# arnauqb/GradABM-JUNE

Measured on NVIDIA B200. Metric: agent_timesteps_per_sec_fwd_bwd, higher is better.
Workload: dtype f32

## Files before the change

### gradabm-june_b200/csrc/gj_kernels.cu

```cuda
#include <cuda_runtime.h>
#include <math.h>
#include <stdint.h>
#include <stdio.h>
#include <stdlib.h>
#include <string.h>

#include "gj_device.cuh"
#include "gj_tiled.cuh"
#include "gj_lean.cuh"
#include "gj_pipe.cuh"

namespace gj {

static thread_local char g_err[512] = "";

static int fail(const char* what, cudaError_t e) {
  snprintf(g_err, sizeof(g_err), "%s: %s", what, cudaGetErrorString(e));
  return -2;
}
static int bad(const char* what) {
  snprintf(g_err, sizeof(g_err), "invalid argument: %s", what);
  return -1;
}
#define GJ_CHECK_LAUNCH(name)                         \
// ... 559 lines not shown
         aligned16(w->orig_id) &&
         aligned16(lp.r_slot) && aligned16(lp.r_pc);
}
static bool pipe_aligned_bwd(const gj_world_desc* w, const LeanPlan& lp, const gj_bwd_io* io) {
  const void* ptrs[] = {io->s, io->inf, io->tinf, io->cur, io->nxt, io->ttn, io->tape_y0, io->tape_v, io->g_s_o,
                        io->g_inf_o, io->g_tinf_o, io->g_cur_o, io->g_nxt_o, io->g_ttn_o, io->prof4, io->g_inf,
                        io->g_tinf, io->T_in, io->w, io->wq, w->ent1, w->cls, lp.r_slot, lp.r_pc};
  for (const void* q : ptrs)
    if (!aligned16(q)) return false;
  return true;
}
template <typename K>
static int pipe_grid(const gj_world_desc* w, K kernel, int threads, size_t smem, OccCache* cache,
                     const Batch& bt = kNoBatch) {
  int& c = cache->v[current_device()];
  if (c == 0) {
    int per_sm = 0;
    cudaFuncSetAttribute(kernel, cudaFuncAttributeMaxDynamicSharedMemorySize, (int)smem);
    if (cudaOccupancyMaxActiveBlocksPerMultiprocessor(&per_sm, kernel, threads, smem) != cudaSuccess || per_sm < 1)
      per_sm = 1;
    c = per_sm;
  }
  const int64_t g = (int64_t)sm_count() * c;
  if (bt.nb > 1) return batch_grid(w, g, bt);
  return (int)(w->n_tiles < g ? w->n_tiles : g);
}

static int check_world(const gj_world_desc* w) {
  if (!w) return bad("world is NULL");
  if (w->n_agents < 0 || w->n_types < 0 || w->n_types > GJ_MAX_TYPES) return bad("world sizes");
  if (w->n_edges >= ((int64_t)1 << 32) || w->n_agents >= ((int64_t)1 << 32)) return bad("world too large for 32-bit CSR");
  for (int t = 0; t < w->n_types; ++t)
    if (w->type_group_off[t + 1] - w->type_group_off[t] >= ((int64_t)1 << 28)) return bad("too many groups in one type");
  return 0;
}

template <bool kBwd>
static int launch_group_pass(const gj_world_desc* w, const gj_step_params* p, const Channels& ch, const float* beta,
                             const float* lprob, const float* in0, const float* in1, float* out_a, float* out_b,
                             const Scratch& sc, cudaStream_t st) {
  if (w->n_small > 0) {
    ProfScope ps(kBwd ? K_GROUP_SMALL_B : K_GROUP_SMALL_F, st);
    k_group_small<kBwd><<<blocks_for(w->n_small, kBlock), kBlock, 0, st>>>(*w, *p, ch, beta, lprob, in0, in1, out_a,
                                                                         out_b);
    GJ_CHECK_LAUNCH("k_group_small");
  }
  if (w->n_chunks > 0) {
    ProfScope ps(kBwd ? K_GROUP_CHUNK_B : K_GROUP_CHUNK_F, st);
    k_group_chunk<kBwd><<<blocks_for(w->n_chunks * 32, kBlock), kBlock, 0, st>>>(*w, *p, ch, beta, lprob, in0, in1,
                                                                              out_a, out_b, sc.part_a, sc.part_b);
    GJ_CHECK_LAUNCH("k_group_chunk");
  }
  if (w->n_big > 0) {
    ProfScope ps(kBwd ? K_GROUP_FIX_B : K_GROUP_FIX_F, st);
    k_group_fix<kBwd><<<blocks_for(w->n_big, kBlock), kBlock, 0, st>>>(*w, *p, ch, beta, sc.part_a, sc.part_b, out_a,
                                                                     out_b);
    GJ_CHECK_LAUNCH("k_group_fix");
  }
  return 0;
}

static int launch_cell_groups(const gj_world_desc* w, const gj_step_params* p, const Plan& pl, const float* beta,
                              float* out_scaled, float* out_plain, const Scratch& sc, cudaStream_t st,
                              const Batch& bt = kNoBatch) {
  if (pl.n_t2 == 0) return 0;
  int64_t maxG = 1;
// ... 47 lines not shown
      lp->c_row[j] = p->nets[k].prob_row;
      lp->c_care[j] = kind == GJ_KIND_CARE_VISIT;
      lp->c_cell_off[j] = w->cell_off[t];
      lp->c_tile_cell[j] = w->tile_cell[t];
      bool seen = false;
      for (int i = 0; i < lp->n_tc; ++i) seen = seen || lp->tc[i] == w->tile_cell[t];
      if (!seen) {
        lp->ctp[lp->n_tc] = w->cell_tile_ptr[t];
        lp->tc[lp->n_tc++] = w->tile_cell[t];
      }
    } else if (kind == GJ_KIND_HOUSEHOLD) {
      if (p->n_quar > 0) return false;
    } else if (kind != GJ_KIND_PLAIN) {
      return false;
    }
  }
  lp->n_cell = pl.n_t2;
  lp->has_generic = pl.n_generic > 0;
  lp->gen_base = total;
  return true;
}

static int launch_lean_group_pass(const gj_world_desc* w, const gj_step_params* p, const Plan& pl, const float* beta,
                                  const float* in, float* out_scaled, float* out_plain, const Scratch& sc, bool bwd,
                                  cudaStream_t st, const Batch& bt);
static int launch_lean_forward_sums(const gj_world_desc* w, const gj_step_params* p, const Plan& pl, const float* beta,
                                    const float* in, float* out_scaled, float* out_plain, const Scratch& sc,
                                    cudaStream_t st, const Batch& bt) {
  if (w->n_giant_chunks > 0) {
    gj_world_desc wg = *w;
    wg.n_small = 0;
    wg.n_chunks = w->n_giant_chunks;
    wg.n_big = w->n_giant_big;
    if (int e = launch_lean_group_pass(&wg, p, pl, beta, in, out_scaled, out_plain, sc, false, st, bt)) return e;
  }
  {
    ProfScope ps(K_GROUP_SMALL_F, st);
    Scatter sct{sc.sct_acc, sc.sct_dirty};
    GenericRanges gr;
    memset(&gr, 0, sizeof(gr));
    for (int t = 0; t < w->n_types; ++t)
      if (w->type_tier[t] == GJ_TIER_GENERIC && w->type_group_off[t + 1] > w->type_group_off[t]) {
        gr.first[gr.n] = w->type_group_off[t];
        gr.start[gr.n + 1] = gr.start[gr.n] + (w->type_group_off[t + 1] - w->type_group_off[t]);
        ++gr.n;
      }
    if (gr.n == 0) return 0;
    launch_pdl(k_lean_scatter_finalize, dim3(blocks_for(gr.start[gr.n], kBlock) * bt.nb), dim3(kBlock), 0, st, *w, *p, pl,
               gr, beta, in, sct, out_scaled, out_plain, bt);
    GJ_CHECK_LAUNCH("k_lean_scatter_finalize");
  }
  return 0;
}

static int launch_lean_group_pass(const gj_world_desc* w, const gj_step_params* p, const Plan& pl, const float* beta,
                                  const float* in, float* out_scaled, float* out_plain, const Scratch& sc, bool bwd,
                                  cudaStream_t st, const Batch& bt) {
  if (w->n_small > 0 || w->n_chunks > 0) {
    ProfScope ps(bwd ? K_GROUP_CHUNK_B : K_GROUP_CHUNK_F, st);
    const int chunk_blocks = w->n_chunks > 0 ? blocks_for(w->n_chunks * 32, kBlock) : 0;
    const int small_blocks = w->n_small > 0 ? blocks_for(w->n_small, kBlock) : 0;
    launch_pdl(k_lean_group_sums, dim3((chunk_blocks + small_blocks) * bt.nb), dim3(kBlock), 0, st, *w, *p, pl, beta, in,
               out_scaled, out_plain, sc.part_a, chunk_blocks, bt);
    GJ_CHECK_LAUNCH("k_lean_group_sums");
  }
  if (w->n_big > 0) {
    ProfScope ps(bwd ? K_GROUP_FIX_B : K_GROUP_FIX_F, st);
    launch_pdl(k_lean_group_fix, dim3(blocks_for(w->n_big * 32, kBlock) * bt.nb), dim3(kBlock), 0, st, *w, *p, pl, beta,
               (const float*)sc.part_a, out_scaled, out_plain, bt);
    GJ_CHECK_LAUNCH("k_lean_group_fix");
  }
  return 0;
}

static int lean_forward(const gj_world_desc* w, const gj_step_params* p, const Plan& pl, const LeanPlan& lp,
                        const gj_fwd_io* io, const Scratch& sc, cudaStream_t st, const NextStep* next,
                        const Batch& bt = kNoBatch) {
  const bool quar = p->n_quar > 0;
  const bool batch = bt.nb > 1;
  if (p->stage != GJ_STAGE_REST) {
    if (!p->t_ready) {
      ProfScope ps(K_TRANSMISSION, st);
      static OccCache occ[4];
      const Scatter sct{sc.sct_acc, sc.sct_dirty};
#define GJ_K1(Q, B, I)                                                                                               \
  launch_pdl(k_lean_transmission<Q, B>, dim3(lean_grid(w, k_lean_transmission<Q, B>, &occ[I], bt)), dim3(kLeanThreads), \
             0, st, *w, *p, lp, *io, sc.tile_part, sct, bt)
#define GJ_K1C(Q, B, I)                                                                                              \
  launch_pdl(k_lean_transmission_c<Q, B>, dim3(lean_grid(w, k_lean_transmission_c<Q, B>, &occ_c[I], bt)),              \
             dim3(kLeanThreads), 0, st, *w, *p, lp, *io, sc.tile_part, sct, bt)
      static OccCache occ_c[4];
      const bool compact = (pipe_flags() & 4) == 0;
      if (compact) {
        if (batch) {
          if (quar) GJ_K1C(true, true, 3);
          else GJ_K1C(false, true, 2);
// ... 811 lines not shown
```

### gradabm-june_b200/csrc/gj_lean.cuh

```cuda
#pragma once
#include "gj_tiled.cuh"

namespace gj {

constexpr int kLeanThreads = 256;
#ifndef GJ_LEAN_MINB_FWD
#define GJ_LEAN_MINB_FWD 3
#endif
#ifndef GJ_LEAN_MINB_BWD
#define GJ_LEAN_MINB_BWD 4
#endif
#ifndef GJ_LEAN_MINB_GATHER
#define GJ_LEAN_MINB_GATHER 3
#endif
constexpr uint32_t kEntNone = 0xFFFFFFFFu;
constexpr uint32_t kEntMulti = 0xFFFFFFFEu;
constexpr uint32_t kEntGiant = 0x80000000u;
constexpr uint32_t kEntId = 0x7FFFFFFFu;

struct Scatter {
  unsigned long long* acc;
  uint8_t* dirty;
};
constexpr float kScatterScale = (float)(1ull << GJ_SCATTER_FRAC);
// ... 434 lines not shown
__device__ __forceinline__ void lean_group_chunk_body(const gj_world_desc& w, const LeanGroupShared& gs, int64_t ci,
                                                      const float* __restrict__ in, float* __restrict__ out_scaled,
                                                      float* __restrict__ out_plain, float* __restrict__ part) {
  const int lane = threadIdx.x & 31;
  if (ci >= w.n_chunks) return;
  const uint32_t g = w.chunk_group[ci];
  const float b = lean_group_beta(gs, g);
  float S = 0.0f;
  if (b == b) {
    const uint32_t j0 = w.chunk_begin[ci], j1 = w.chunk_end[ci];
    constexpr int kDeep = 4;
    for (uint32_t j = j0 + lane; j < j1; j += 32 * kDeep) {
      uint32_t m[kDeep];
      float x[kDeep];
#pragma unroll
      for (int k = 0; k < kDeep; ++k) m[k] = (j + 32 * k < j1) ? w.gm_agent[j + 32 * k] : 0u;
#pragma unroll
      for (int k = 0; k < kDeep; ++k) x[k] = (j + 32 * k < j1) ? in[m[k]] : 0.0f;
#pragma unroll
      for (int k = 0; k < kDeep; ++k) S += x[k];
    }
    S = warp_sum(S);
  }
  if (lane != 0) return;
  const int pi = w.chunk_part[ci];
  if (pi < 0) {
    out_plain[g] = S;
    out_scaled[g] = (b == b) ? (b * w.pc[g]) * S : 0.0f;
  } else {
    part[pi] = S;
  }
}

__global__ void __launch_bounds__(kBlock) k_lean_group_sums(gj_world_desc w, gj_step_params p, Plan pl,
                                                            const float* __restrict__ beta,
                                                            const float* __restrict__ in, float* __restrict__ out_scaled,
                                                            float* __restrict__ out_plain, float* __restrict__ part,
                                                            int chunk_blocks, Batch bt) {
  __shared__ LeanGroupShared gs;
  pdl_launch();
  pdl_wait();
  uint32_t bx = blockIdx.x;
  if (bt.nb > 1) {
    const int s = (int)(bx % (uint32_t)bt.nb);
    bx /= (uint32_t)bt.nb;
    beta += (int64_t)s * bt.sBeta;
    in += (int64_t)s * bt.sN;
    out_scaled += (int64_t)s * bt.sG;
    out_plain += (int64_t)s * bt.sG;
    part = scr_shift(part, bt, s);
  }
  lean_beta_sums(gs, w, p, pl, beta);
  if ((int)bx < chunk_blocks)
    lean_group_chunk_body(w, gs, ((int64_t)bx * blockDim.x + threadIdx.x) >> 5, in, out_scaled, out_plain, part);
  else
    lean_group_small_body(w, gs, (int64_t)(bx - chunk_blocks) * blockDim.x + threadIdx.x, in, out_scaled,
                          out_plain);
}

__global__ void __launch_bounds__(kBlock) k_lean_group_fix(gj_world_desc w, gj_step_params p, Plan pl,
                                                           const float* __restrict__ beta,
                                                           const float* __restrict__ part,
                                                           float* __restrict__ out_scaled,
                                                           float* __restrict__ out_plain, Batch bt) {
  __shared__ LeanGroupShared gs;
  pdl_launch();
  pdl_wait();
  uint32_t bx = blockIdx.x;
  if (bt.nb > 1) {
    const int s = (int)(bx % (uint32_t)bt.nb);
    bx /= (uint32_t)bt.nb;
    beta += (int64_t)s * bt.sBeta;
    out_scaled += (int64_t)s * bt.sG;
    out_plain += (int64_t)s * bt.sG;
    part = scr_shift(part, bt, s);
  }
  lean_beta_sums(gs, w, p, pl, beta);
  const int lane = threadIdx.x & 31;
  const int64_t i = ((int64_t)bx * blockDim.x + threadIdx.x) >> 5;
  if (i >= w.n_big) return;
  const uint32_t g = w.big_groups[i];
  const float b = lean_group_beta(gs, g);
  float S = 0.0f;
  for (uint32_t j = w.big_part_ptr[i] + lane; j < w.big_part_ptr[i + 1]; j += 32) S += part[j];
  S = warp_sum(S);
  if (lane != 0) return;
  out_plain[g] = S;
  out_scaled[g] = (b == b) ? (b * w.pc[g]) * S : 0.0f;
}

// ... 597 lines not shown
```

### gradabm-june_b200/csrc/gj_world.cu

```cuda
#include <cuda_runtime.h>
#include <stdint.h>
#include <stdio.h>
#include <string.h>

#include <string>
#include <vector>

#include <thrust/adjacent_difference.h>
#include <thrust/binary_search.h>
#include <thrust/copy.h>
#include <thrust/count.h>
#include <thrust/device_ptr.h>
#include <thrust/device_vector.h>
#include <thrust/extrema.h>
#include <thrust/fill.h>
#include <thrust/gather.h>
#include <thrust/host_vector.h>
#include <thrust/iterator/counting_iterator.h>
#include <thrust/iterator/zip_iterator.h>
#include <thrust/tuple.h>
#include <thrust/reduce.h>
#include <thrust/scan.h>
#include <thrust/scatter.h>
#include <thrust/sequence.h>
// ... 108 lines not shown
    thrust::copy(b.begin(), b.end(), out.begin() + a.size());
    return out;
  }
  static I64 select(const I64& v, const I64& mask) { return gather(v, nonzero(mask)); }
  static I64 unique_inverse(const I64& keys, int64_t* n_unique) {
    const int64_t n = (int64_t)keys.size();
    I64 k = keys;
    I64 perm = arange(n);
    thrust::sort_by_key(k.begin(), k.end(), perm.begin());
    I64 fresh(n, 0);
    if (n > 0) {
      thrust::transform(k.begin() + 1, k.end(), k.begin(), fresh.begin() + 1,
                        [] __host__ __device__(int64_t a, int64_t b) { return (int64_t)(a != b); });
      thrust::inclusive_scan(fresh.begin(), fresh.end(), fresh.begin());
    }
    I64 rank(n);
    thrust::scatter(fresh.begin(), fresh.end(), perm.begin(), rank.begin());
    *n_unique = n > 0 ? (int64_t)fresh.back() + 1 : 0;
    return rank;
  }
};

struct TypeSrc {
  std::string name;
  int64_t E, G;
};

template <class B>
struct World {
  template <class T>
  using vec = typename B::template vec<T>;
  gj_world_desc desc;
  vec<uint32_t> am_ptr, am_ent, gm_ptr, gm_agent, small_groups, chunk_group, chunk_begin, chunk_end, big_groups,
      big_part_ptr, tile_begin, tile_flags, ent1, orig_id;
  vec<int32_t> chunk_part;
  vec<float> pc;
  vec<uint8_t> cls;
  vec<uint32_t> range_slot[GJ_MAX_TYPES];
  vec<float> range_pc[GJ_MAX_TYPES];
  vec<uint32_t> tile_cell[GJ_MAX_TYPES], cell_tile_ptr[GJ_MAX_TYPES], cell_grp_ptr[GJ_MAX_TYPES], cell_grp[GJ_MAX_TYPES],
      grp_cell_ptr[GJ_MAX_TYPES], grp_cell[GJ_MAX_TYPES];
  vec<int64_t> perm;
  std::string error;
};

template <class B>
struct Builder {
  using O = Ops<B>;
  using I64 = typename O::I64;
  template <class T>
  using vec = typename B::template vec<T>;

  static vec<uint32_t> to_u32(const I64& v, int slack = 0) {
    vec<uint32_t> out(v.size() + slack, 0u);
    thrust::transform(v.begin(), v.end(), out.begin(), [] __host__ __device__(int64_t x) { return (uint32_t)x; });
    return out;
  }
  template <class T>
  static const T* raw(const vec<T>& v) {
    return v.empty() ? nullptr : thrust::raw_pointer_cast(v.data());
  }

  struct Cell {
    int64_t n_cells = 0;
    I64 cell_start, cell_of_agent, cell_grp_ptr, cell_grp, grp_cell_ptr, grp_cell;
  };

// ... 291 lines not shown
  for (int t = 0; t < nt; ++t) {
    if (s->want_tier) want[t] = s->want_tier[t];
    else if (t == range_type) want[t] = GJ_TIER_RANGE;
    else if (t == cell_type) want[t] = GJ_TIER_CELL;
  }
  std::vector<typename Bd::Cell> cells(nt);
  std::vector<int> tier(nt, GJ_TIER_GENERIC);
  I64 g_src, g_key, g_ent;
  for (int t = 0; t < nt; ++t) {
    if (n > 0 && want[t] == GJ_TIER_RANGE) {
      I64 slot;
      typename B::template vec<float> rpc;
      bool from_size = false;
      if (Bd::try_range(n, src[t], dst[t], types[t].G, W->pc, offs[t], &slot, &rpc, &from_size)) {
        tier[t] = GJ_TIER_RANGE;
        d.range_pc_from_size[t] = from_size ? 1 : 0;
        W->range_slot[t] = Bd::to_u32(slot, 32);
        W->range_pc[t] = rpc;
      }
    } else if (n > 0 && want[t] == GJ_TIER_CELL) {
      if (Bd::try_cell(n, src[t], dst[t], types[t].G, &cells[t])) tier[t] = GJ_TIER_CELL;
    }
    if (tier[t] == GJ_TIER_GENERIC) {
      const int64_t off = offs[t], tt = t;
      g_src = O::cat(g_src, src[t]);
      g_key = O::cat(g_key, O::map1(dst[t], [off] __host__ __device__(int64_t g) { return g + off; }));
      g_ent = O::cat(g_ent, O::map1(dst[t], [tt] __host__ __device__(int64_t g) { return g + (tt << 28); }));
    }
  }
  const int64_t E = (int64_t)g_src.size();

  I64 size = O::bincount(g_key, G);
  I64 gm_ptr = O::ptr_from_counts(size);
  {
    I64 perm = O::argsort_stable(g_key);
    W->gm_agent = Bd::to_u32(O::gather(g_src, perm));
  }
  I64 deg = O::bincount(g_src, n);
  I64 am_ptr = O::ptr_from_counts(deg);
  {
    I64 perm = O::argsort_stable(g_src);
    W->am_ent = Bd::to_u32(O::gather(g_ent, perm), 32);
  }
  {
    I64 ent1(n, kNoSlot);
    I64 v = O::map2(g_key, O::gather(size, g_key), [scatter_max] __host__ __device__(int64_t k, int64_t sz) {
      return k + ((int64_t)(sz > scatter_max) << 31);
    });
    O::scatter(ent1, g_src, v);
    thrust::transform(ent1.begin(), ent1.end(), deg.begin(), ent1.begin(),
                      [] __host__ __device__(int64_t e, int64_t dg) { return dg > 1 ? kEntMulti : e; });
    W->ent1 = Bd::to_u32(ent1, 32);
  }
  {
    typename B::template vec<uint8_t> cls(n + 64, (uint8_t)0);
    thrust::transform(sex.begin(), sex.end(), age.begin(), cls.begin(),
                      [] __host__ __device__(int64_t sx, int64_t ag) { return (uint8_t)(sx * 100 + ag); });
    W->cls = cls;
  }

  I64 generic_group(G, 0);
  for (int t = 0; t < nt; ++t)
    if (tier[t] == GJ_TIER_GENERIC) thrust::fill(generic_group.begin() + offs[t], generic_group.begin() + offs[t + 1], (int64_t)1);
  I64 gids = O::arange(G);
  I64 small_mask = O::map2(size, generic_group, [small_group] __host__ __device__(int64_t sz, int64_t g) { return (int64_t)(sz <= small_group && g); });
  I64 big_giant = O::map2(size, generic_group, [small_group, scatter_max] __host__ __device__(int64_t sz, int64_t g) { return (int64_t)(sz > small_group && sz > scatter_max && g); });
  I64 big_rest = O::map2(size, generic_group, [small_group, scatter_max] __host__ __device__(int64_t sz, int64_t g) { return (int64_t)(sz > small_group && sz <= scatter_max && g); });
  I64 small = O::select(gids, small_mask);
  I64 bg_g = O::select(gids, big_giant);
  I64 bg = O::cat(bg_g, O::select(gids, big_rest));
  const int64_t n_giant_big = (int64_t)bg_g.size();
  I64 nchunk = O::map1(O::gather(size, bg), [chunk] __host__ __device__(int64_t sz) { return (sz + chunk - 1) / chunk; });
  int64_t n_giant_chunks = 0;
  if (n_giant_big > 0) n_giant_chunks = thrust::reduce(nchunk.begin(), nchunk.begin() + n_giant_big, (int64_t)0);
  I64 cfirst = O::ptr_from_counts(nchunk);
  I64 cseg = O::segments(cfirst);
  I64 chunk_group = O::gather(bg, cseg);
  const int64_t n_chunks = (int64_t)chunk_group.size();
  I64 within = O::map2(O::arange(n_chunks), O::gather(cfirst, cseg), [] __host__ __device__(int64_t i, int64_t f) { return i - f; });
  I64 chunk_begin = O::map2(O::gather(gm_ptr, chunk_group), within, [chunk] __host__ __device__(int64_t p, int64_t w) { return p + w * chunk; });
  I64 cg1 = O::map1(chunk_group, [] __host__ __device__(int64_t g) { return g + 1; });
  I64 chunk_end = O::map2(chunk_begin, O::gather(gm_ptr, cg1), [chunk] __host__ __device__(int64_t b, int64_t e) { return b + chunk < e ? b + chunk : e; });
  I64 multi_g = O::map1(nchunk, [] __host__ __device__(int64_t c) { return (int64_t)(c > 1); });
  I64 multi = O::gather(multi_g, cseg);
  I64 part_idx(n_chunks, 0);
  thrust::exclusive_scan(multi.begin(), multi.end(), part_idx.begin());
  const int64_t n_parts = O::sum_of(multi);
  {
    typename B::template vec<int32_t> chunk_part(n_chunks);
    thrust::transform(multi.begin(), multi.end(), part_idx.begin(), chunk_part.begin(),
                      [] __host__ __device__(int64_t m, int64_t i) { return m ? (int32_t)i : (int32_t)-1; });
    W->chunk_part = chunk_part;
  }
  I64 big_groups = O::select(bg, multi_g);
  I64 big_part_ptr = O::ptr_from_counts(O::select(nchunk, multi_g));

  I64 cuts(1, 0);
  for (int t = 0; t < nt; ++t)
    if (tier[t] == GJ_TIER_CELL) cuts = O::cat(cuts, cells[t].cell_start);
  I64 tile_begin;
  if (n > 0) {
    thrust::sort(cuts.begin(), cuts.end());
    cuts.resize(thrust::unique(cuts.begin(), cuts.end()) - cuts.begin());
    I64 seg_start = cuts;
    I64 seg_end(seg_start.size());
    thrust::copy(seg_start.begin() + 1, seg_start.end(), seg_end.begin());
    seg_end[seg_end.size() - 1] = n;
    const int64_t T = GJ_TILE_AGENTS;
    I64 ntile = O::map2(seg_end, seg_start, [T] __host__ __device__(int64_t e, int64_t b) { return (e - b + T - 1) / T; });
    I64 tfirst = O::ptr_from_counts(ntile);
    I64 tseg = O::segments(tfirst);
    const int64_t n_tiles = (int64_t)tseg.size();
    I64 tw = O::map2(O::arange(n_tiles), O::gather(tfirst, tseg), [] __host__ __device__(int64_t i, int64_t f) { return i - f; });
    tile_begin = O::map2(O::gather(seg_start, tseg), tw, [T] __host__ __device__(int64_t b, int64_t w) { return b + w * T; });
    tile_begin.push_back(n);
  } else {
    tile_begin = I64(1, 0);
  }
  const int64_t n_tiles = (int64_t)tile_begin.size() - 1;
  I64 tile_flags(n_tiles, 0);
  if (n_tiles > 0) tile_flags[0] = 1;
  int64_t cell_off = 0;
  for (int t = 0; t < nt; ++t) {
    d.type_tier[t] = tier[t];
    d.cell_off[t] = cell_off;
    if (tier[t] == GJ_TIER_RANGE) {
      d.range_slot[t] = Bd::raw(W->range_slot[t]);
      d.range_pc[t] = Bd::raw(W->range_pc[t]);
// ... 5 lines not shown
        thrust::transform(thrust::make_zip_iterator(thrust::make_tuple(tc.begin() + 1, tc.begin(), tile_flags.begin() + 1)),
                          thrust::make_zip_iterator(thrust::make_tuple(tc.end(), tc.end() - 1, tile_flags.end())),
                          tile_flags.begin() + 1, [] __host__ __device__(thrust::tuple<int64_t, int64_t, int64_t> x) {
                            return thrust::get<2>(x) | (int64_t)(thrust::get<0>(x) != thrust::get<1>(x));
                          });
      W->tile_cell[t] = Bd::to_u32(tc);
      I64 ctp = O::searchsorted_left(tb0, c.cell_start);
      ctp.push_back(n_tiles);
      W->cell_tile_ptr[t] = Bd::to_u32(ctp);
      W->cell_grp_ptr[t] = Bd::to_u32(c.cell_grp_ptr);
      W->cell_grp[t] = Bd::to_u32(c.cell_grp);
      W->grp_cell_ptr[t] = Bd::to_u32(c.grp_cell_ptr);
      W->grp_cell[t] = Bd::to_u32(c.grp_cell);
      d.n_cells[t] = c.n_cells;
      d.tile_cell[t] = Bd::raw(W->tile_cell[t]);
      d.cell_tile_ptr[t] = Bd::raw(W->cell_tile_ptr[t]);
      d.cell_grp_ptr[t] = Bd::raw(W->cell_grp_ptr[t]);
      d.cell_grp[t] = Bd::raw(W->cell_grp[t]);
      d.grp_cell_ptr[t] = Bd::raw(W->grp_cell_ptr[t]);
      d.grp_cell[t] = Bd::raw(W->grp_cell[t]);
      cell_off += c.n_cells;
    }
  }
  d.n_cells_total = cell_off;

  W->am_ptr = Bd::to_u32(am_ptr, 32);
  W->gm_ptr = Bd::to_u32(gm_ptr);
  W->small_groups = Bd::to_u32(small);
  W->chunk_group = Bd::to_u32(chunk_group);
  W->chunk_begin = Bd::to_u32(chunk_begin);
  W->chunk_end = Bd::to_u32(chunk_end);
  W->big_groups = Bd::to_u32(big_groups);
  W->big_part_ptr = Bd::to_u32(big_part_ptr);
  W->tile_begin = Bd::to_u32(tile_begin, 4);
  W->tile_flags = Bd::to_u32(tile_flags, 4);
  if (!orig.empty()) W->orig_id = Bd::to_u32(orig, 32);

  d.n_agents = n;
  d.n_groups = G;
  d.n_edges = n_edges_total;
  d.n_types = nt;
  for (int t = 0; t <= nt; ++t) d.type_group_off[t] = offs[t];
  d.am_ptr = Bd::raw(W->am_ptr);
  d.am_ent = Bd::raw(W->am_ent);
  d.gm_ptr = Bd::raw(W->gm_ptr);
  d.gm_agent = Bd::raw(W->gm_agent);
  d.pc = Bd::raw(W->pc);
  d.cls = Bd::raw(W->cls);
  d.small_groups = Bd::raw(W->small_groups);
  d.n_small = (int64_t)small.size();
  d.chunk_group = Bd::raw(W->chunk_group);
  d.chunk_begin = Bd::raw(W->chunk_begin);
  d.chunk_end = Bd::raw(W->chunk_end);
  d.chunk_part = Bd::raw(W->chunk_part);
  d.n_chunks = n_chunks;
  d.big_groups = Bd::raw(W->big_groups);
  d.big_part_ptr = Bd::raw(W->big_part_ptr);
  d.n_big = (int64_t)big_groups.size();
  d.n_parts = n_parts;
  d.n_tiles = n_tiles;
  d.tile_begin = Bd::raw(W->tile_begin);
  d.tile_flags = Bd::raw(W->tile_flags);
  d.ent1 = Bd::raw(W->ent1);
  d.n_giant_chunks = n_giant_chunks;
  d.n_giant_big = n_giant_big;
  d.dbeta_w = nullptr;
  d.orig_id = Bd::raw(W->orig_id);
  (void)E;
  return 0;
}

}

struct gj_world {
  gjw::World<gjw::DeviceBackend>* dev = nullptr;
  gjw::World<gjw::HostBackend>* host = nullptr;
  thrust::host_vector<int64_t> perm_host;
};

static thread_local char g_world_err[512] = "";

extern "C" {

const char* gj_world_last_error(void) { return g_world_err; }

static int build_any(const gj_world_src* src, gj_world** out, bool on_device) {
  if (!src || !out) {
    snprintf(g_world_err, sizeof(g_world_err), "gj_world_build: NULL argument");
    return -1;
  }
  gj_world* w = new gj_world();
  int rc = 0;
// ... 62 lines not shown
```

### gradabm-june_b200/grad_june/_lib.py

```python
import ctypes as C
import os
import subprocess
from pathlib import Path

PKG_DIR = Path(__file__).resolve().parent
CSRC_DIR = PKG_DIR.parent / "csrc"
INCLUDE_DIR = PKG_DIR.parent.parent / "include"
LIB_PATH = Path(os.environ.get("GJ_LIB_PATH") or PKG_DIR / "libgradjune_b200.so")

GJ_MAX_TYPES = 8
GJ_MAX_NETS = 16
GJ_MAX_STAGES = 16
GJ_MAX_QUAR = 4
GJ_MAX_AGE_BINS = 8
GJ_MAX_CHANNELS = 8
GJ_ABI_VERSION = 10

KIND_PLAIN, KIND_HOUSEHOLD, KIND_LEISURE, KIND_CARE_VISIT = 0, 1, 2, 3
PHASE_NETWORKS, PHASE_SAMPLE, PHASE_INFECT, PHASE_SYMPTOMS, PHASE_ALL = 1, 2, 4, 8, 15
MODE_STEP, MODE_SEED = 0, 1
STAGE_ALL, STAGE_SUMS, STAGE_REST = 0, 1, 2

_u32p = C.c_void_p
_f32p = C.c_void_p


class WorldDesc(C.Structure):
    _fields_ = [
        ("n_agents", C.c_int64), ("n_groups", C.c_int64), ("n_edges", C.c_int64),
        ("n_types", C.c_int32), ("_pad0", C.c_int32),
        ("type_group_off", C.c_int64 * (GJ_MAX_TYPES + 1)),
        ("am_ptr", _u32p), ("am_ent", _u32p), ("gm_ptr", _u32p), ("gm_agent", _u32p),
        ("pc", _f32p), ("cls", C.c_void_p),
        ("small_groups", _u32p), ("n_small", C.c_int64),
        ("chunk_group", _u32p), ("chunk_begin", _u32p), ("chunk_end", _u32p), ("chunk_part", C.c_void_p),
        ("n_chunks", C.c_int64),
        ("big_groups", _u32p), ("big_part_ptr", _u32p), ("n_big", C.c_int64), ("n_parts", C.c_int64),
        ("type_tier", C.c_int32 * GJ_MAX_TYPES),
        ("range_slot", C.c_void_p * GJ_MAX_TYPES), ("range_pc", C.c_void_p * GJ_MAX_TYPES),
        ("range_pc_from_size", C.c_int32 * GJ_MAX_TYPES),
        ("n_tiles", C.c_int64), ("tile_begin", _u32p), ("tile_flags", _u32p),
        ("n_cells", C.c_int64 * GJ_MAX_TYPES), ("cell_off", C.c_int64 * GJ_MAX_TYPES), ("n_cells_total", C.c_int64),
        ("tile_cell", C.c_void_p * GJ_MAX_TYPES), ("cell_tile_ptr", C.c_void_p * GJ_MAX_TYPES),
        ("cell_grp_ptr", C.c_void_p * GJ_MAX_TYPES), ("cell_grp", C.c_void_p * GJ_MAX_TYPES),
        ("grp_cell_ptr", C.c_void_p * GJ_MAX_TYPES), ("grp_cell", C.c_void_p * GJ_MAX_TYPES),
        ("ent1", _u32p), ("n_giant_chunks", C.c_int64), ("n_giant_big", C.c_int64), ("dbeta_w", _f32p), ("orig_id", _u32p),
    ]


class WorldSrc(C.Structure):
    _fields_ = [
        ("n_agents", C.c_int64), ("n_types", C.c_int32), ("renumber", C.c_int32),
        ("type_name", C.c_char_p * GJ_MAX_TYPES),
        ("edge_agent", C.c_void_p * GJ_MAX_TYPES), ("edge_group", C.c_void_p * GJ_MAX_TYPES),
        ("n_edges", C.c_int64 * GJ_MAX_TYPES), ("n_groups", C.c_int64 * GJ_MAX_TYPES),
        ("people_i64", C.c_void_p * GJ_MAX_TYPES), ("people_f32", C.c_void_p * GJ_MAX_TYPES),
        ("age", C.c_void_p), ("sex", C.c_void_p), ("original_index", C.c_void_p), ("want_tier", C.c_void_p),
    ]


class Net(C.Structure):
    _fields_ = [("type", C.c_int32), ("kind", C.c_int32), ("prob_row", C.c_int32), ("s_off", C.c_int32)]


class Dist(C.Structure):
    _fields_ = [("kind", C.c_int32), ("loc", C.c_float), ("scale", C.c_float)]


class StepParams(C.Structure):
    _fields_ = [
# ... 199 lines not shown
```

### gradabm-june_b200/grad_june/world.py

```python
import io
import pickle
import sys
from typing import Dict, List, Optional

import numpy as np
import torch

MAX_TYPES = 8


class _Store:
    def __init__(self, key=None):
        object.__setattr__(self, "_mapping", {})
        object.__setattr__(self, "_key", key)

    def __getattr__(self, name):
        if name.startswith("__"):
            raise AttributeError(name)
        mapping = self.__dict__.get("_mapping", {})
        if name in mapping:
            return mapping[name]
        raise AttributeError(f"{type(self).__name__} {self.__dict__.get('_key')!r} has no attribute {name!r}")

    def __setattr__(self, name, value):
# ... 151 lines not shown


def load_world(path_or_file):
    if hasattr(path_or_file, "read"):
        return _WorldUnpickler(path_or_file).load()
    with open(path_or_file, "rb") as f:
        return _WorldUnpickler(f).load()


def world_from_arrays(arrays: Dict[str, np.ndarray], types: List[str], device="cpu") -> HeteroData:
    data = HeteroData()
    n = len(arrays["age"])
    data["agent"].id = torch.arange(n)
    data["agent"].age = torch.as_tensor(np.asarray(arrays["age"]).astype(np.int64))
    data["agent"].sex = torch.as_tensor(np.asarray(arrays["sex"]).astype(np.int64))
    if "ethnicity" in arrays:
        data["agent"].ethnicity = np.asarray(arrays["ethnicity"])
    for t in types:
        ng = int(arrays[f"{t}_ngroups"])
        data[t].id = torch.arange(ng)
        data[t].people = torch.as_tensor(np.asarray(arrays[f"{t}_people"]).astype(np.int64))
        ei = np.stack([arrays[f"{t}_src"], arrays[f"{t}_dst"]]).astype(np.int64)
        data["agent", "attends_" + t, t].edge_index = torch.as_tensor(ei)
    data = ToUndirected()(data)
    return data.to(device)


TIER_GENERIC, TIER_RANGE, TIER_CELL = 0, 1, 2
TILE_AGENTS = 1024
RANGE_MAX_GROUP = 64
CELL_MIN_MEAN_AGENTS = 64
CELL_MAX_GROUPS = 16
SCATTER_MAX_GROUP = 32768


class DeviceWorld:

    def __init__(self, **kw):
        self.__dict__.update(kw)

    def desc(self):
        from . import _lib

        d = self.__dict__.get("_desc")
        if d is not None:
            return d
        d = _lib.WorldDesc()
        d.n_agents, d.n_groups, d.n_edges, d.n_types = self.n_agents, self.n_groups, self.n_edges, len(self.types)
        for i, off in enumerate(self.type_group_off):
            d.type_group_off[i] = off
        for name in ("am_ptr", "am_ent", "gm_ptr", "gm_agent", "pc", "cls", "small_groups", "chunk_group",
                     "chunk_begin", "chunk_end", "chunk_part", "big_groups", "big_part_ptr", "tile_begin", "tile_flags",
                     "ent1"):
            setattr(d, name, getattr(self, name).data_ptr())
        d.n_small, d.n_chunks = self.small_groups.numel(), self.chunk_group.numel()
        d.n_big, d.n_parts = self.big_groups.numel(), self.n_parts
        d.n_giant_chunks, d.n_giant_big = self.__dict__.get("n_giant_chunks", 0), self.__dict__.get("n_giant_big", 0)
        d.n_tiles = self.tile_begin.numel() - 1
        cell_off = 0
        for ti in range(len(self.types)):
            d.type_tier[ti] = self.type_tier[ti]
            d.cell_off[ti] = cell_off
            if self.type_tier[ti] == TIER_RANGE:
                d.range_slot[ti] = self.range_slot[ti].data_ptr()
                d.range_pc[ti] = self.range_pc[ti].data_ptr()
                d.range_pc_from_size[ti] = 1 if self.__dict__.get("range_pc_from_size", {}).get(ti) else 0
            elif self.type_tier[ti] == TIER_CELL:
                c = self.cells[ti]
                d.n_cells[ti] = c["n_cells"]
                for name in ("tile_cell", "cell_tile_ptr", "cell_grp_ptr", "cell_grp", "grp_cell_ptr", "grp_cell"):
                    getattr(d, name)[ti] = c[name].data_ptr()
                cell_off += c["n_cells"]
        d.n_cells_total = cell_off
        if self.__dict__.get("dbeta_w") is not None:
            d.dbeta_w = self.dbeta_w.data_ptr()
        if self.__dict__.get("orig_id") is not None:
            d.orig_id = self.orig_id.data_ptr()
        self.__dict__["_desc"] = d
        return d


def p_contact(people: torch.Tensor) -> torch.Tensor:
    one = torch.tensor(1.0, device=people.device)
    zero = torch.tensor(0.0, device=people.device)
    return torch.maximum(torch.minimum(1.0 / (people - 1), one), zero).to(torch.float32)


def _u32(t):
# ... 263 lines not shown
        src = gkey = ent = torch.zeros(0, dtype=torch.long, device=dev)
    E = src.numel()
    if n_edges_total >= (1 << 32) or n_agents >= (1 << 32):
        raise ValueError("world too large for 32-bit CSR offsets")
    _, perm = torch.sort(gkey, stable=True)
    gm_agent = src[perm].to(torch.int32)
    size = torch.bincount(gkey, minlength=G) if E else torch.zeros(G, dtype=torch.long, device=dev)
    gm_ptr = _ptr_from_counts(size)
    del perm
    _, perm = torch.sort(src, stable=True)
    am_ent = ent[perm].to(torch.int64)
    deg = torch.bincount(src, minlength=n_agents) if E else torch.zeros(n_agents, dtype=torch.long, device=dev)
    am_ptr = _ptr_from_counts(deg)
    del perm
    if G >= (1 << 31):
        raise ValueError("too many groups for the one-entry-per-agent view")
    if scatter_max < chunk:
        raise ValueError("scatter_max must be at least one chunk")
    ent1 = torch.full((n_agents,), 0xFFFFFFFF, dtype=torch.long, device=dev)
    if E:
        ent1[src] = gkey + ((size[gkey] > scatter_max).long() << 31)
        ent1[deg > 1] = 0xFFFFFFFE
    age = age.to(dev).long()
    sex = sex.to(dev).long()
    if age.numel() and (int(age.min()) < 0 or int(age.max()) > 99 or int(sex.min()) < 0 or int(sex.max()) > 1):
        raise ValueError("age must be in [0, 99] and sex in {0, 1}")
    cls = (sex * 100 + age).to(torch.uint8)

    generic_group = torch.zeros(G, dtype=torch.bool, device=dev)
    for ti in range(len(types)):
        if type_tier[ti] == TIER_GENERIC:
            generic_group[offs[ti]:offs[ti + 1]] = True
    gids = torch.arange(G, device=dev)
    small = gids[(size <= small_group) & generic_group]
    big_mask = (size > small_group) & generic_group
    giant = size > scatter_max
    bg = torch.cat((gids[big_mask & giant], gids[big_mask & ~giant]))
    n_giant_big = int((big_mask & giant).sum())
    nchunk = (size[bg] + chunk - 1) // chunk
    n_giant_chunks = int(nchunk[:n_giant_big].sum())
    chunk_group = torch.repeat_interleave(bg, nchunk)
    first = _ptr_from_counts(nchunk)
    within = torch.arange(chunk_group.numel(), device=dev) - torch.repeat_interleave(first[:-1], nchunk)
    chunk_begin = gm_ptr[chunk_group] + within * chunk
    chunk_end = torch.minimum(chunk_begin + chunk, gm_ptr[chunk_group + 1])
    multi = torch.repeat_interleave(nchunk > 1, nchunk)
    chunk_part = torch.full((chunk_group.numel(),), -1, dtype=torch.long, device=dev)
    n_parts = int(multi.sum())
    chunk_part[multi] = torch.arange(n_parts, device=dev)
    big_groups = bg[nchunk > 1]
    big_part_ptr = _ptr_from_counts(nchunk[nchunk > 1])

    cuts = [torch.zeros(1, dtype=torch.long, device=dev)]
    for c in cells.values():
        cuts.append(c["cell_start"])
    seg_start = torch.unique(torch.cat(cuts)) if n_agents > 0 else torch.zeros(0, dtype=torch.long, device=dev)
    seg_end = torch.cat((seg_start[1:], torch.tensor([n_agents], device=dev))) if n_agents > 0 else seg_start
    ntile = (seg_end - seg_start + TILE_AGENTS - 1) // TILE_AGENTS
    tfirst = _ptr_from_counts(ntile)
    tw = torch.arange(int(ntile.sum()), device=dev) - torch.repeat_interleave(tfirst[:-1], ntile)
    tile_begin = torch.cat((torch.repeat_interleave(seg_start, ntile) + tw * TILE_AGENTS,
                            torch.tensor([n_agents], device=dev)))
    tile_flags = torch.zeros(tile_begin.numel() - 1, dtype=torch.long, device=dev)
    if tile_flags.numel():
        tile_flags[0] = 1
    for ti, c in cells.items():
        tc = c["cell_of_agent"][tile_begin[:-1]]
        tile_flags[1:] |= (tc[1:] != tc[:-1]).long()
    for ti, c in cells.items():
        c["tile_cell"] = _u32(c["cell_of_agent"][tile_begin[:-1]])
        c["cell_tile_ptr"] = _u32(torch.cat((torch.searchsorted(tile_begin[:-1].contiguous(), c["cell_start"]),
                                             torch.tensor([tile_begin.numel() - 1], device=dev))))
        del c["cell_of_agent"]

    return DeviceWorld(
        n_agents=n_agents, n_groups=G, n_edges=n_edges_total, n_generic_edges=E, types=list(types),
        type_group_off=offs, type_tier=type_tier, range_slot=range_slot, range_pc=range_pc, cells=cells,
        range_pc_from_size=range_from_size,
        group_size=size, am_ptr=_padded(_u32(am_ptr)), am_ent=_padded(_u32(am_ent)), gm_ptr=_u32(gm_ptr),
        gm_agent=gm_agent.contiguous(), pc=pc.contiguous(), cls=_padded(cls.contiguous(), 64), small_groups=_u32(small),
        chunk_group=_u32(chunk_group), chunk_begin=_u32(chunk_begin), chunk_end=_u32(chunk_end),
        chunk_part=chunk_part.to(torch.int32), big_groups=_u32(big_groups), big_part_ptr=_u32(big_part_ptr),
        n_parts=n_parts, tile_begin=_padded(_u32(tile_begin), 4), tile_flags=_padded(_u32(tile_flags), 4),
        ent1=_padded(_u32(ent1)), device=dev,
        orig_id=None if orig_id is None else _padded(_u32(orig_id.to(dev))),
        n_giant_chunks=n_giant_chunks, n_giant_big=n_giant_big,
    )


class NativeWorld:

    def __init__(self, data: "HeteroData", device="cuda:0", renumber=True, host=False, want_tiers=None):
        import ctypes as C

        from . import _lib
        L = _lib.lib()
        dev = torch.device("cpu" if host else device)
        types = data.venue_types()
        src = _lib.WorldSrc()
        keep = []

        def ptr(t, dtype):
            t = torch.as_tensor(t).to(device=dev, dtype=dtype).contiguous()
            keep.append(t)
            return t.data_ptr()

        n = len(data["agent"].id)
        src.n_agents, src.n_types, src.renumber = n, len(types), 1 if renumber else 0
        for i, t in enumerate(types):
            ei = data["attends_" + t].edge_index
            src.type_name[i] = t.encode()
            src.edge_agent[i], src.edge_group[i] = ptr(ei[0], torch.long), ptr(ei[1], torch.long)
            src.n_edges[i], src.n_groups[i] = ei.shape[1], len(data[t]["id"])
            people = torch.as_tensor(data[t]["people"])
            if people.dtype.is_floating_point:
                src.people_f32[i] = ptr(people, torch.float32)
            else:
# ... 302 lines not shown
```

### include/gradjune_b200.h

```cpp
#ifndef GRADJUNE_B200_H
#define GRADJUNE_B200_H

#include <stddef.h>
#include <stdint.h>

#ifdef __cplusplus
extern "C" {
#endif

#define GJ_ABI_VERSION 10

#define GJ_MAX_TYPES 8
#define GJ_MAX_NETS 16
#define GJ_MAX_STAGES 16
#define GJ_MAX_QUAR 4
#define GJ_MAX_AGE_BINS 8
#define GJ_MAX_CHANNELS 8

#define GJ_SMALL_GROUP 16
#define GJ_CHUNK 1024

#define GJ_SCATTER_MAX_GROUP 32768
#define GJ_SCATTER_CAP_LOG2 10
#define GJ_SCATTER_FRAC 37

enum { GJ_TIER_GENERIC = 0, GJ_TIER_RANGE = 1, GJ_TIER_CELL = 2 };
#define GJ_TILE_AGENTS 1024
#define GJ_MAX_RANGE_NETS 4

enum { GJ_KIND_PLAIN = 0, GJ_KIND_HOUSEHOLD = 1, GJ_KIND_LEISURE = 2, GJ_KIND_CARE_VISIT = 3 };

enum {
  GJ_PHASE_NETWORKS = 1,
  GJ_PHASE_SAMPLE = 2,
  GJ_PHASE_INFECT = 4,
  GJ_PHASE_SYMPTOMS = 8,
  GJ_PHASE_ALL = 15
};

enum { GJ_STAGE_ALL = 0, GJ_STAGE_SUMS = 1, GJ_STAGE_REST = 2 };

enum {
  GJ_MODE_STEP = 0,
  GJ_MODE_SEED = 1
};

typedef struct gj_world_desc {
  int64_t n_agents;
  int64_t n_groups;
  int64_t n_edges;
  int32_t n_types;
  int32_t _pad0;
  int64_t type_group_off[GJ_MAX_TYPES + 1];

  const uint32_t* am_ptr;
  const uint32_t* am_ent;

  const uint32_t* gm_ptr;
  const uint32_t* gm_agent;
  const float* pc;

  const uint8_t* cls;

  const uint32_t* small_groups;
  int64_t n_small;
  const uint32_t* chunk_group;
  const uint32_t* chunk_begin;
  const uint32_t* chunk_end;
  const int32_t* chunk_part;
  int64_t n_chunks;
  const uint32_t* big_groups;
  const uint32_t* big_part_ptr;
  int64_t n_big;
  int64_t n_parts;

  int32_t type_tier[GJ_MAX_TYPES];
  const uint32_t* range_slot[GJ_MAX_TYPES];
  const float* range_pc[GJ_MAX_TYPES];
  int32_t range_pc_from_size[GJ_MAX_TYPES];
  int64_t n_tiles;
  const uint32_t* tile_begin;
  const uint32_t* tile_flags;
  int64_t n_cells[GJ_MAX_TYPES];
  int64_t cell_off[GJ_MAX_TYPES];
  int64_t n_cells_total;
  const uint32_t* tile_cell[GJ_MAX_TYPES];
  const uint32_t* cell_tile_ptr[GJ_MAX_TYPES];
  const uint32_t* cell_grp_ptr[GJ_MAX_TYPES];
  const uint32_t* cell_grp[GJ_MAX_TYPES];
  const uint32_t* grp_cell_ptr[GJ_MAX_TYPES];
  const uint32_t* grp_cell[GJ_MAX_TYPES];
  const uint32_t* ent1;
  int64_t n_giant_chunks;
  int64_t n_giant_big;
  const float* dbeta_w;
  const uint32_t* orig_id;
} gj_world_desc;

typedef struct gj_world_src {
  int64_t n_agents;
  int32_t n_types;
  int32_t renumber;
  const char* type_name[GJ_MAX_TYPES];
  const int64_t* edge_agent[GJ_MAX_TYPES];
  const int64_t* edge_group[GJ_MAX_TYPES];
  int64_t n_edges[GJ_MAX_TYPES];
  int64_t n_groups[GJ_MAX_TYPES];
// ... 187 lines not shown
```

Measured before the change: 21.19 billion.

## Sort group-sum work by agent locality and run it as persistent blocks

Small and chunked generic groups are reordered by the id of each group's middle member. A precomputed sum_block schedule interleaves chunk and small blocks in that agent order, and the group-sum kernel now runs as a persistent, occupancy-sized grid that walks the schedule with a prefetched next entry. The goal is better cache locality on the agent-indexed reads and less launch/tail overhead. The cost is extra world-build sorting, a new ABI field, and a per-block beta-sum prologue that is now amortized over many units.

```diff
diff --git a/gradabm-june_b200/csrc/gj_kernels.cu b/gradabm-june_b200/csrc/gj_kernels.cu
--- a/gradabm-june_b200/csrc/gj_kernels.cu
+++ b/gradabm-june_b200/csrc/gj_kernels.cu
@@ -615,6 +615,7 @@
   if (w->n_edges >= ((int64_t)1 << 32) || w->n_agents >= ((int64_t)1 << 32)) return bad("world too large for 32-bit CSR");
   for (int t = 0; t < w->n_types; ++t)
     if (w->type_group_off[t + 1] - w->type_group_off[t] >= ((int64_t)1 << 28)) return bad("too many groups in one type");
+  if ((w->n_small > 0 || w->n_chunks > 0) && (!w->sum_block || w->n_sum_blocks <= 0)) return bad("world has no sum_block");
   return 0;
 }
 
@@ -728,6 +729,7 @@
     wg.n_small = 0;
     wg.n_chunks = w->n_giant_chunks;
     wg.n_big = w->n_giant_big;
+    wg.n_sum_blocks = blocks_for(w->n_giant_chunks * 32, kBlock);
     if (int e = launch_lean_group_pass(&wg, p, pl, beta, in, out_scaled, out_plain, sc, false, st, bt)) return e;
   }
   {
@@ -752,12 +754,18 @@
 static int launch_lean_group_pass(const gj_world_desc* w, const gj_step_params* p, const Plan& pl, const float* beta,
                                   const float* in, float* out_scaled, float* out_plain, const Scratch& sc, bool bwd,
                                   cudaStream_t st, const Batch& bt) {
-  if (w->n_small > 0 || w->n_chunks > 0) {
+  if (w->n_sum_blocks > 0) {
     ProfScope ps(bwd ? K_GROUP_CHUNK_B : K_GROUP_CHUNK_F, st);
-    const int chunk_blocks = w->n_chunks > 0 ? blocks_for(w->n_chunks * 32, kBlock) : 0;
-    const int small_blocks = w->n_small > 0 ? blocks_for(w->n_small, kBlock) : 0;
-    launch_pdl(k_lean_group_sums, dim3((chunk_blocks + small_blocks) * bt.nb), dim3(kBlock), 0, st, *w, *p, pl, beta, in,
-               out_scaled, out_plain, sc.part_a, chunk_blocks, bt);
+    static OccCache occ;
+    int& per_sm = occ.v[current_device()];
+    if (per_sm == 0 && (cudaOccupancyMaxActiveBlocksPerMultiprocessor(&per_sm, k_lean_group_sums, kBlock, 0) !=
+                            cudaSuccess || per_sm < 1))
+      per_sm = 1;
+    int64_t units = (int64_t)sm_count() * per_sm / bt.nb;
+    if (units < 1) units = 1;
+    if (units > w->n_sum_blocks) units = w->n_sum_blocks;
+    launch_pdl(k_lean_group_sums, dim3((unsigned)(units * bt.nb)), dim3(kBlock), 0, st, *w, *p, pl, beta, in,
+               out_scaled, out_plain, sc.part_a, bt);
     GJ_CHECK_LAUNCH("k_lean_group_sums");
   }
   if (w->n_big > 0) {
diff --git a/gradabm-june_b200/csrc/gj_lean.cuh b/gradabm-june_b200/csrc/gj_lean.cuh
--- a/gradabm-june_b200/csrc/gj_lean.cuh
+++ b/gradabm-june_b200/csrc/gj_lean.cuh
@@ -490,18 +490,20 @@
   }
 }
 
+static_assert(kBlock == GJ_GROUP_SUM_THREADS, "w.sum_block is built for blocks of GJ_GROUP_SUM_THREADS threads");
 __global__ void __launch_bounds__(kBlock) k_lean_group_sums(gj_world_desc w, gj_step_params p, Plan pl,
                                                             const float* __restrict__ beta,
                                                             const float* __restrict__ in, float* __restrict__ out_scaled,
                                                             float* __restrict__ out_plain, float* __restrict__ part,
-                                                            int chunk_blocks, Batch bt) {
+                                                            Batch bt) {
   __shared__ LeanGroupShared gs;
   pdl_launch();
   pdl_wait();
-  uint32_t bx = blockIdx.x;
+  uint32_t bx = blockIdx.x, nbx = gridDim.x;
   if (bt.nb > 1) {
     const int s = (int)(bx % (uint32_t)bt.nb);
     bx /= (uint32_t)bt.nb;
+    nbx /= (uint32_t)bt.nb;
     beta += (int64_t)s * bt.sBeta;
     in += (int64_t)s * bt.sN;
     out_scaled += (int64_t)s * bt.sG;
@@ -509,11 +511,16 @@
     part = scr_shift(part, bt, s);
   }
   lean_beta_sums(gs, w, p, pl, beta);
-  if ((int)bx < chunk_blocks)
-    lean_group_chunk_body(w, gs, ((int64_t)bx * blockDim.x + threadIdx.x) >> 5, in, out_scaled, out_plain, part);
-  else
-    lean_group_small_body(w, gs, (int64_t)(bx - chunk_blocks) * blockDim.x + threadIdx.x, in, out_scaled,
-                          out_plain);
+  uint32_t e = bx < w.n_sum_blocks ? w.sum_block[bx] : 0u;
+  for (int64_t u = bx; u < w.n_sum_blocks; u += nbx) {
+    const uint32_t cur = e;
+    if (u + nbx < w.n_sum_blocks) e = w.sum_block[u + nbx];
+    const int64_t t = (int64_t)(cur & 0x7FFFFFFFu) * blockDim.x + threadIdx.x;
+    if (cur >> 31)
+      lean_group_small_body(w, gs, t, in, out_scaled, out_plain);
+    else
+      lean_group_chunk_body(w, gs, t >> 5, in, out_scaled, out_plain, part);
+  }
 }
 
 __global__ void __launch_bounds__(kBlock) k_lean_group_fix(gj_world_desc w, gj_step_params p, Plan pl,
diff --git a/gradabm-june_b200/csrc/gj_world.cu b/gradabm-june_b200/csrc/gj_world.cu
--- a/gradabm-june_b200/csrc/gj_world.cu
+++ b/gradabm-june_b200/csrc/gj_world.cu
@@ -164,7 +164,7 @@
   using vec = typename B::template vec<T>;
   gj_world_desc desc;
   vec<uint32_t> am_ptr, am_ent, gm_ptr, gm_agent, small_groups, chunk_group, chunk_begin, chunk_end, big_groups,
-      big_part_ptr, tile_begin, tile_flags, ent1, orig_id;
+      big_part_ptr, sum_block, tile_begin, tile_flags, ent1, orig_id;
   vec<int32_t> chunk_part;
   vec<float> pc;
   vec<uint8_t> cls;
@@ -522,9 +522,14 @@
 
   I64 size = O::bincount(g_key, G);
   I64 gm_ptr = O::ptr_from_counts(size);
+  I64 key;
   {
     I64 perm = O::argsort_stable(g_key);
-    W->gm_agent = Bd::to_u32(O::gather(g_src, perm));
+    I64 gm_agent = O::gather(g_src, perm);
+    W->gm_agent = Bd::to_u32(gm_agent);
+    I64 lo(gm_ptr.begin(), gm_ptr.end() - 1), hi(gm_ptr.begin() + 1, gm_ptr.end());
+    I64 mid = O::map2(lo, hi, [E] __host__ __device__(int64_t b, int64_t e) { return b < e ? (b + e) / 2 : E; });
+    key = O::gather(O::cat(gm_agent, I64(1, 0)), mid);
   }
   I64 deg = O::bincount(g_src, n);
   I64 am_ptr = O::ptr_from_counts(deg);
@@ -557,8 +562,10 @@
   I64 big_giant = O::map2(size, generic_group, [small_group, scatter_max] __host__ __device__(int64_t sz, int64_t g) { return (int64_t)(sz > small_group && sz > scatter_max && g); });
   I64 big_rest = O::map2(size, generic_group, [small_group, scatter_max] __host__ __device__(int64_t sz, int64_t g) { return (int64_t)(sz > small_group && sz <= scatter_max && g); });
   I64 small = O::select(gids, small_mask);
+  small = O::gather(small, O::argsort_stable(O::gather(key, small)));
   I64 bg_g = O::select(gids, big_giant);
-  I64 bg = O::cat(bg_g, O::select(gids, big_rest));
+  I64 rest = O::select(gids, big_rest);
+  I64 bg = O::cat(bg_g, O::gather(rest, O::argsort_stable(O::gather(key, rest))));
   const int64_t n_giant_big = (int64_t)bg_g.size();
   I64 nchunk = O::map1(O::gather(size, bg), [chunk] __host__ __device__(int64_t sz) { return (sz + chunk - 1) / chunk; });
   int64_t n_giant_chunks = 0;
@@ -584,6 +591,15 @@
   }
   I64 big_groups = O::select(bg, multi_g);
   I64 big_part_ptr = O::ptr_from_counts(O::select(nchunk, multi_g));
+  const int64_t per_cb = GJ_GROUP_SUM_THREADS / 32, per_sb = GJ_GROUP_SUM_THREADS;
+  const int64_t n_gb = (n_giant_chunks + per_cb - 1) / per_cb;
+  I64 cb = O::arange((n_chunks + per_cb - 1) / per_cb - n_gb, n_gb);
+  I64 sb = O::arange(((int64_t)small.size() + per_sb - 1) / per_sb);
+  I64 cfirst_item = O::map1(cb, [per_cb] __host__ __device__(int64_t b) { return b * per_cb; });
+  I64 sfirst_item = O::map1(sb, [per_sb] __host__ __device__(int64_t b) { return b * per_sb; });
+  I64 bkey = O::cat(O::gather(key, O::gather(chunk_group, cfirst_item)), O::gather(key, O::gather(small, sfirst_item)));
+  I64 blk = O::cat(cb, O::map1(sb, [] __host__ __device__(int64_t b) { return b | ((int64_t)1 << 31); }));
+  I64 sum_block = O::cat(O::arange(n_gb), O::gather(blk, O::argsort_stable(bkey)));
 
   I64 cuts(1, 0);
   for (int t = 0; t < nt; ++t)
@@ -655,6 +671,7 @@
   W->chunk_end = Bd::to_u32(chunk_end);
   W->big_groups = Bd::to_u32(big_groups);
   W->big_part_ptr = Bd::to_u32(big_part_ptr);
+  W->sum_block = Bd::to_u32(sum_block);
   W->tile_begin = Bd::to_u32(tile_begin, 4);
   W->tile_flags = Bd::to_u32(tile_flags, 4);
   if (!orig.empty()) W->orig_id = Bd::to_u32(orig, 32);
@@ -681,6 +698,8 @@
   d.big_part_ptr = Bd::raw(W->big_part_ptr);
   d.n_big = (int64_t)big_groups.size();
   d.n_parts = n_parts;
+  d.sum_block = Bd::raw(W->sum_block);
+  d.n_sum_blocks = (int64_t)sum_block.size();
   d.n_tiles = n_tiles;
   d.tile_begin = Bd::raw(W->tile_begin);
   d.tile_flags = Bd::raw(W->tile_flags);
diff --git a/gradabm-june_b200/grad_june/_lib.py b/gradabm-june_b200/grad_june/_lib.py
--- a/gradabm-june_b200/grad_june/_lib.py
+++ b/gradabm-june_b200/grad_june/_lib.py
@@ -14,7 +14,7 @@
 GJ_MAX_QUAR = 4
 GJ_MAX_AGE_BINS = 8
 GJ_MAX_CHANNELS = 8
-GJ_ABI_VERSION = 10
+GJ_ABI_VERSION = 11
 
 KIND_PLAIN, KIND_HOUSEHOLD, KIND_LEISURE, KIND_CARE_VISIT = 0, 1, 2, 3
 PHASE_NETWORKS, PHASE_SAMPLE, PHASE_INFECT, PHASE_SYMPTOMS, PHASE_ALL = 1, 2, 4, 8, 15
@@ -36,6 +36,7 @@
         ("chunk_group", _u32p), ("chunk_begin", _u32p), ("chunk_end", _u32p), ("chunk_part", C.c_void_p),
         ("n_chunks", C.c_int64),
         ("big_groups", _u32p), ("big_part_ptr", _u32p), ("n_big", C.c_int64), ("n_parts", C.c_int64),
+        ("sum_block", _u32p), ("n_sum_blocks", C.c_int64),
         ("type_tier", C.c_int32 * GJ_MAX_TYPES),
         ("range_slot", C.c_void_p * GJ_MAX_TYPES), ("range_pc", C.c_void_p * GJ_MAX_TYPES),
         ("range_pc_from_size", C.c_int32 * GJ_MAX_TYPES),
diff --git a/gradabm-june_b200/grad_june/world.py b/gradabm-june_b200/grad_june/world.py
--- a/gradabm-june_b200/grad_june/world.py
+++ b/gradabm-june_b200/grad_june/world.py
@@ -207,6 +207,7 @@
 CELL_MIN_MEAN_AGENTS = 64
 CELL_MAX_GROUPS = 16
 SCATTER_MAX_GROUP = 32768
+GROUP_SUM_THREADS = 256
 
 
 class DeviceWorld:
@@ -225,10 +226,10 @@
         for i, off in enumerate(self.type_group_off):
             d.type_group_off[i] = off
         for name in ("am_ptr", "am_ent", "gm_ptr", "gm_agent", "pc", "cls", "small_groups", "chunk_group",
-                     "chunk_begin", "chunk_end", "chunk_part", "big_groups", "big_part_ptr", "tile_begin", "tile_flags",
-                     "ent1"):
+                     "chunk_begin", "chunk_end", "chunk_part", "big_groups", "big_part_ptr", "sum_block", "tile_begin",
+                     "tile_flags", "ent1"):
             setattr(d, name, getattr(self, name).data_ptr())
-        d.n_small, d.n_chunks = self.small_groups.numel(), self.chunk_group.numel()
+        d.n_small, d.n_chunks, d.n_sum_blocks = self.small_groups.numel(), self.chunk_group.numel(), self.sum_block.numel()
         d.n_big, d.n_parts = self.big_groups.numel(), self.n_parts
         d.n_giant_chunks, d.n_giant_big = self.__dict__.get("n_giant_chunks", 0), self.__dict__.get("n_giant_big", 0)
         d.n_tiles = self.tile_begin.numel() - 1
@@ -558,10 +559,17 @@
         if type_tier[ti] == TIER_GENERIC:
             generic_group[offs[ti]:offs[ti + 1]] = True
     gids = torch.arange(G, device=dev)
+    key = torch.zeros(G, dtype=torch.long, device=dev)
+    if E:
+        filled = size > 0
+        key[filled] = gm_agent[((gm_ptr[:-1] + gm_ptr[1:]) // 2)[filled]].long()
     small = gids[(size <= small_group) & generic_group]
+    small = small[torch.sort(key[small], stable=True)[1]]
     big_mask = (size > small_group) & generic_group
     giant = size > scatter_max
-    bg = torch.cat((gids[big_mask & giant], gids[big_mask & ~giant]))
+    rest = gids[big_mask & ~giant]
+    rest = rest[torch.sort(key[rest], stable=True)[1]]
+    bg = torch.cat((gids[big_mask & giant], rest))
     n_giant_big = int((big_mask & giant).sum())
     nchunk = (size[bg] + chunk - 1) // chunk
     n_giant_chunks = int(nchunk[:n_giant_big].sum())
@@ -576,6 +584,13 @@
     chunk_part[multi] = torch.arange(n_parts, device=dev)
     big_groups = bg[nchunk > 1]
     big_part_ptr = _ptr_from_counts(nchunk[nchunk > 1])
+    per_cb = GROUP_SUM_THREADS // 32
+    n_gb = (n_giant_chunks + per_cb - 1) // per_cb
+    cb = torch.arange(n_gb, (chunk_group.numel() + per_cb - 1) // per_cb, device=dev)
+    sb = torch.arange((small.numel() + GROUP_SUM_THREADS - 1) // GROUP_SUM_THREADS, device=dev)
+    bkey = torch.cat((key[chunk_group[cb * per_cb]], key[small[sb * GROUP_SUM_THREADS]]))
+    rest_blocks = torch.cat((cb, sb | (1 << 31)))[torch.sort(bkey, stable=True)[1]]
+    sum_block = torch.cat((torch.arange(n_gb, device=dev), rest_blocks))
 
     cuts = [torch.zeros(1, dtype=torch.long, device=dev)]
     for c in cells.values():
@@ -607,8 +622,8 @@
         gm_agent=gm_agent.contiguous(), pc=pc.contiguous(), cls=_padded(cls.contiguous(), 64), small_groups=_u32(small),
         chunk_group=_u32(chunk_group), chunk_begin=_u32(chunk_begin), chunk_end=_u32(chunk_end),
         chunk_part=chunk_part.to(torch.int32), big_groups=_u32(big_groups), big_part_ptr=_u32(big_part_ptr),
-        n_parts=n_parts, tile_begin=_padded(_u32(tile_begin), 4), tile_flags=_padded(_u32(tile_flags), 4),
-        ent1=_padded(_u32(ent1)), device=dev,
+        n_parts=n_parts, sum_block=_u32(sum_block), tile_begin=_padded(_u32(tile_begin), 4),
+        tile_flags=_padded(_u32(tile_flags), 4), ent1=_padded(_u32(ent1)), device=dev,
         orig_id=None if orig_id is None else _padded(_u32(orig_id.to(dev))),
         n_giant_chunks=n_giant_chunks, n_giant_big=n_giant_big,
     )
diff --git a/include/gradjune_b200.h b/include/gradjune_b200.h
--- a/include/gradjune_b200.h
+++ b/include/gradjune_b200.h
@@ -8,7 +8,7 @@
 extern "C" {
 #endif
 
-#define GJ_ABI_VERSION 10
+#define GJ_ABI_VERSION 11
 
 #define GJ_MAX_TYPES 8
 #define GJ_MAX_NETS 16
@@ -19,6 +19,7 @@
 
 #define GJ_SMALL_GROUP 16
 #define GJ_CHUNK 1024
+#define GJ_GROUP_SUM_THREADS 256
 
 #define GJ_SCATTER_MAX_GROUP 32768
 #define GJ_SCATTER_CAP_LOG2 10
@@ -73,6 +74,8 @@
   const uint32_t* big_part_ptr;
   int64_t n_big;
   int64_t n_parts;
+  const uint32_t* sum_block;
+  int64_t n_sum_blocks;
 
   int32_t type_tier[GJ_MAX_TYPES];
   const uint32_t* range_slot[GJ_MAX_TYPES];
```

Result: faster. 21.64 billion (median of 6 runs) (+2.1%).
